# MCG-NJU/MotionRAG

Hardware: AMD Instinct MI355X
Metric: denoise_step_frames_per_sec (higher is better)
Workload: dtype bf16

## Files before the change

### include/mrag_hip.h

```cpp
#ifndef MRAG_HIP_H
#define MRAG_HIP_H

#include <stdint.h>

#ifdef __cplusplus
extern "C" {
#endif

#define MRAG_OK 0
#define MRAG_EINVAL (-1)
#define MRAG_ENOTSUP (-2)

int mrag_abi_version(void);
const char* mrag_target_arch(void);
const char* mrag_source_hash(void);

enum mrag_kernel_id {
  MRAG_K_GEMM_W4 = 0,
  MRAG_K_GEMM_W4_QKNORM_ROPE,
  MRAG_K_GEMM_W4_GEGLU,
  MRAG_K_GEMM_256x256,
  MRAG_K_GEMM_256x320,
  MRAG_K_GEMM_256x128,
  MRAG_K_GEMM_128x128,
// ... 69 lines not shown
  float qk_eps, q_premul;
  int32_t qk_first;
  int32_t tuning;
  int32_t geglu_act;
  void* workspace;
  float acc_scale;
  int64_t workspace_bytes;
  int64_t w_batch_stride;
  const void* a_ln_gamma; const void* a_ln_beta;
  float a_ln_eps; int32_t a_ln;
} mrag_gemm_args;
enum { MRAG_GEMM_TUNE_NO_WIDE = 1, MRAG_GEMM_TUNE_NO_STAGED = 2, MRAG_GEMM_TUNE_GEGLU_NO_STAGED = 4, MRAG_GEMM_TUNE_STREAMK = 8,
       MRAG_GEMM_TUNE_NO_W4 = 1 << 16,
       MRAG_GEMM_TUNE_NO_SKINNY = 1 << 17,
       MRAG_GEMM_TUNE_SKINNY_8 = 1 << 18,
       MRAG_GEMM_TUNE_TAIL_RECT = 1 << 19  };

int mrag_gemm_bf16(void* stream, const mrag_gemm_args* args);
int64_t mrag_gemm_workspace_bytes(int64_t M, int64_t N, int64_t K);

int mrag_quant_rows_e4m3(void* stream, const void* x, void* x8, int32_t* exp, int64_t M, int64_t K, int64_t ldx, int64_t ld8);

typedef struct mrag_gemm_fp8_args {
  const void* A8;
  const void* W8;
  const int32_t* a_exp;
  const int32_t* w_exp;
  const void* bias;
  void* C;
  const void* resid;
  const void* gate0;
  const void* gate1;
  int64_t M, N, K;
// ... 267 lines not shown
```

### motionrag_amd/attn_processor.py

```python
from __future__ import annotations

from typing import Optional

import torch
from torch import nn

from . import ops
from .layers import WeightCache, linear_resid


def packed_score_layout(heads: int, keys: int):
    tiles32 = -(-(heads * 32) // 256)
    for c in range(keys + (keys & 1), 32, 2):
        if -(-((heads - 1) * c + 32) // 256) < tiles32 and all(((c * h) & 7) + keys <= 32 for h in range(min(heads, 8))):
            return c, -(-((heads - 1) * c + 32) // 256) * 256
    return 32, heads * 32


PACK_SCORE_BLOCKS = True
FOLD_IP_QUERY = True


class Attention(nn.Module):

    def __init__(self, query_dim: int, cross_attention_dim: Optional[int] = None, heads: int = 8, dim_head: int = 64, bias: bool = False,
                 out_bias: bool = True, qk_norm: Optional[str] = None, eps: float = 1e-5, processor=None):
        super().__init__()
        inner = heads * dim_head
        self.heads, self.inner_dim = heads, inner
        self.is_cross_attention = cross_attention_dim is not None
        kv_dim = cross_attention_dim if cross_attention_dim is not None else query_dim
        self.to_q = nn.Linear(query_dim, inner, bias=bias)
        self.to_k = nn.Linear(kv_dim, inner, bias=bias)
        self.to_v = nn.Linear(kv_dim, inner, bias=bias)
        self.to_out = nn.ModuleList([nn.Linear(inner, query_dim, bias=out_bias), nn.Dropout(0.0)])
# ... 23 lines not shown

def _joint_sdpa(q, k, v, fp8_attn: bool):
    if fp8_attn and ops.fp8_joint_attention_supported(q.shape[1], k.shape[1]):
        return ops.joint_attention_fp8(q, k, v, q_prescaled=True)
    return ops.attention(q, k, v, q_prescaled=True)


def joint_attention_core(attn, proc, x: torch.Tensor, text_len: int, rope, ip_hidden_states: Optional[torch.Tensor], scale: float, sp=None,
                         fp8_qkv: bool = False, fp8_attn: bool = False):
    B, S, D = x.shape
    H = attn.heads
    fw = proc._fused
    qkv_lins = (attn.to_q, attn.to_k, attn.to_v)
    wqkv, bqkv = fw.get("qkv", tuple(m.weight for m in qkv_lins) + tuple(m.bias for m in qkv_lins),
                        lambda: (_cat_weights(qkv_lins), _cat_weights(qkv_lins, "bias")))
    cos = sin = None
    if rope is not None:
        cos, sin = fw.get("rope", (rope[0], rope[1]), lambda: tuple(t.to(device=x.device, dtype=torch.float32).contiguous() for t in rope[:2]))
        if getattr(attn, "is_cross_attention", False):
            raise NotImplementedError("RoPE on Q only (is_cross_attention=True) is not used by CogVideoX attn1")
    nq, nk = getattr(attn, "norm_q", None), getattr(attn, "norm_k", None)
    if sp is not None:
        o = _sharded_attention(attn, x, wqkv, bqkv, H, nq, nk, cos, sin, text_len, sp, fp8_attn)
        return _motion_branch(attn, proc, o, ip_hidden_states, scale)
    if fp8_qkv:
        w8, w_exp = fw.get("qkv8", tuple(m.weight for m in qkv_lins), lambda: ops.quant_rows_e4m3(wqkv))
        qkv = ops.linear_fp8(x, w8, w_exp, bqkv)
        ops.qknorm_rope_(qkv, H, nq.weight if nq is not None else None, nq.bias if nq is not None else None, nk.weight if nk is not None else None,
                         nk.bias if nk is not None else None, cos, sin, text_len, eps=nq.eps if nq is not None else 1e-6, q_premul=ops.LOG2E * 64 ** -0.5)
        q5 = qkv.view(B, S, 3, H, 64)
        o = _joint_sdpa(q5[:, :, 0], q5[:, :, 1], q5[:, :, 2], fp8_attn)
        return _motion_branch(attn, proc, o, ip_hidden_states, scale)
    qkv = ops.qkv_linear_qknorm_rope(x, wqkv, bqkv, H, nq.weight if nq is not None else None, nq.bias if nq is not None else None,
                                     nk.weight if nk is not None else None, nk.bias if nk is not None else None, cos, sin, text_len,
                                     eps=nq.eps if nq is not None else 1e-6, q_premul=ops.LOG2E * 64 ** -0.5)
    q5 = qkv.view(B, S, 3, H, 64)
    o = _joint_sdpa(q5[:, :, 0], q5[:, :, 1], q5[:, :, 2], fp8_attn)
    return _motion_branch(attn, proc, o, ip_hidden_states, scale)


def _sharded_attention(attn, x, wqkv, bqkv, H, nq, nk, cos, sin, text_len, sp, fp8_attn=False):
    B, S, D = x.shape
    qn = dict(eps=nq.eps if nq is not None else 1e-6, q_premul=ops.LOG2E * 64 ** -0.5)
    gq, bq, gk, bk = (nq.weight if nq is not None else None, nq.bias if nq is not None else None,
                      nk.weight if nk is not None else None, nk.bias if nk is not None else None)
    try:
        kv = ops.qkv_linear_qknorm_rope(x, wqkv[D:], bqkv[D:] if bqkv is not None else None, H, gq, bq, gk, bk, cos, sin, text_len, first=1, **qn)
    except NotImplementedError:
        qkv = ops.qkv_linear_qknorm_rope(x, wqkv, bqkv, H, gq, bq, gk, bk, cos, sin, text_len, **qn)
        g = sp.all_gather_rows_async(qkv[..., D:].contiguous()).wait().view(B, -1, 2, H, 64)
# ... 156 lines not shown
```

### motionrag_amd/csrc/gemm_bf16.hip

```cpp
#include "gemm_common.h"

namespace {

inline bool skinny_applies(const mrag_gemm_args* a, int epi) {
  const long long row_tiles = (a->M + SKM_ROWS - 1) / SKM_ROWS;
  return a->M <= 256 && row_tiles * a->N * a->K <= 8LL * 4096 * 2048 && a->K >= 256 && a->N >= 256 &&
         !(a->tuning & MRAG_GEMM_TUNE_NO_SKINNY) && ((a->tuning >> 4) & 0xf) == 0 &&
         (epi == MRAG_EPI_NONE || epi == MRAG_EPI_GELU_TANH || epi == MRAG_EPI_GELU_ERF || epi == MRAG_EPI_SILU || epi == MRAG_EPI_RESID) &&
         (!a->bias || (((uintptr_t)a->bias) & 7) == 0);
}

inline bool k320_applies(const mrag_gemm_args* a, int epi) {
  return a->K == 320 && a->N % 320 == 0 && a->N <= 960 && a->M >= 16384 && (epi == MRAG_EPI_NONE || epi == MRAG_EPI_RESID) &&
         !(a->tuning & (MRAG_GEMM_TUNE_NO_WIDE | MRAG_GEMM_TUNE_NO_STAGED | MRAG_GEMM_TUNE_GEGLU_NO_STAGED | MRAG_GEMM_TUNE_STREAMK)) &&
         rows_16B_aligned(a->C, a->ldc, a->resid, a->ldr) && (!a->bias || (((uintptr_t)a->bias) & 7) == 0);
}

}

extern "C" int mrag_gemm_bf16(void* stream, const mrag_gemm_args* a) {
  if (!a || !a->A || !a->W || !a->C) return MRAG_EINVAL;
  if (a->M <= 0 || a->N <= 0 || a->K <= 0) return MRAG_EINVAL;
  if (a->K % 64 != 0 || a->N % 4 != 0) return MRAG_ENOTSUP;
  if (a->epilogue == MRAG_EPI_GEGLU && a->N % 32 != 0) return MRAG_ENOTSUP;
  if (a->lda % 8 != 0 || a->ldw % 8 != 0 || a->ldc % 4 != 0) return MRAG_EINVAL;
  if (((uintptr_t)a->A | (uintptr_t)a->W) & 15) return MRAG_EINVAL;
  if ((uintptr_t)a->C & 7) return MRAG_EINVAL;
  if ((a->epilogue == MRAG_EPI_RESID || a->epilogue == MRAG_EPI_GATE_RESID) &&
      (!a->resid || a->ldr % 4 != 0 || ((uintptr_t)a->resid & 7)))
    return MRAG_EINVAL;
  if (a->epilogue == MRAG_EPI_GATE_RESID &&
      (!a->gate0 || !a->gate1 || a->rows_per_batch <= 0 || a->gate_stride % 4 != 0)) return MRAG_EINVAL;
  GemmP p{};
  p.A = (const bf16_t*)a->A; p.W = (const bf16_t*)a->W; p.bias = (const bf16_t*)a->bias;
  p.C = (bf16_t*)a->C; p.resid = (const bf16_t*)a->resid;
// ... 3 lines not shown
  p.acc_scale = a->acc_scale == 0.0f ? 1.0f : a->acc_scale;
  if (a->w_batch_stride < 0 || a->w_batch_stride % 8 != 0) return MRAG_EINVAL;
  if (a->a_ln != 0 && a->a_ln != 1) return MRAG_EINVAL;
  if (a->a_ln) {
    if ((((uintptr_t)a->a_ln_gamma | (uintptr_t)a->a_ln_beta) & 15) || a->K > 8192) return MRAG_EINVAL;
    p.lna = 1; p.lna_g = (const bf16_t*)a->a_ln_gamma; p.lna_b = (const bf16_t*)a->a_ln_beta; p.lna_eps = a->a_ln_eps;
  }
  p.w_bstride = a->w_batch_stride;
  if (a->epilogue == MRAG_EPI_GEGLU && a->geglu_act != 0 && a->geglu_act != 1) return MRAG_EINVAL;
  if (a->epilogue == MRAG_EPI_QKNORM_ROPE) {
    if (a->qk_dmodel <= 0 || a->qk_dmodel % 64 != 0 || a->N % a->qk_dmodel != 0 || a->qk_first < 0 || a->qk_first + a->N / a->qk_dmodel > 3 ||
        a->rows_per_batch <= 0) return MRAG_EINVAL;
    if ((a->rope_cos != nullptr) != (a->rope_sin != nullptr) || (((uintptr_t)a->rope_cos | (uintptr_t)a->rope_sin) & 15)) return MRAG_EINVAL;
    if (((uintptr_t)a->q_gamma | (uintptr_t)a->q_beta | (uintptr_t)a->k_gamma | (uintptr_t)a->k_beta) & 15) return MRAG_EINVAL;
    p.qg = (const bf16_t*)a->q_gamma; p.qb = (const bf16_t*)a->q_beta; p.kg = (const bf16_t*)a->k_gamma; p.kb = (const bf16_t*)a->k_beta;
    p.rcos = a->rope_cos; p.rsin = a->rope_sin; p.qk_D = a->qk_dmodel; p.rope_text_len = a->rope_text_len; p.qk_first = a->qk_first; p.qk_eps = a->qk_eps; p.q_premul = a->q_premul;
  }
  hipStream_t s = (hipStream_t)stream;
  const long long t256 = ((a->M + 255) / 256) * ((a->N + 255) / 256);
  p.tuning = a->tuning;
  const int epi = (a->epilogue == MRAG_EPI_GEGLU && a->geglu_act == 1) ? EPI_GEGLU_TANH : a->epilogue;
  if (const int cfg = (a->tuning >> 4) & 0xf) {
    if (cfg == 1 && t256 >= 192) return launch_tiled(s, p, epi, TILE_256x256_W16, nullptr);
    if (cfg == 2) return launch_tiled(s, p, epi, TILE_128x128, nullptr);
    if (cfg == 4 || (cfg == 3 && t256 >= 192)) {
      const int rc = launch_w4(s, p, epi);
      if (rc != MRAG_ENOTSUP) return rc;
    }
  }
  if (a->w_batch_stride != 0) {
    if (epi != MRAG_EPI_NONE || a->N % 128 != 0 || a->K < 320 || a->rows_per_batch <= 0 || a->M % a->rows_per_batch != 0 || a->ldc % 8 != 0 || (((uintptr_t)a->C) & 15) ||
        (a->tuning & (MRAG_GEMM_TUNE_NO_W4 | MRAG_GEMM_TUNE_NO_STAGED)))
      return MRAG_ENOTSUP;
    return launch_w4(s, p, epi);
  }
  if (a->a_ln) return skinny_applies(a, epi) ? launch_skinny(s, p, epi) : MRAG_ENOTSUP;
  if (skinny_applies(a, epi)) return launch_skinny(s, p, epi);
  if (k320_applies(a, epi)) return launch_k320(s, p, epi);
  const bool w4_ok = t256 >= 192 && !(a->tuning & (MRAG_GEMM_TUNE_NO_W4 | MRAG_GEMM_TUNE_NO_STAGED | MRAG_GEMM_TUNE_STREAMK | MRAG_GEMM_TUNE_NO_WIDE)) && a->N % 128 == 0 &&
// ... 16 lines not shown
    if (pl.use && a->workspace_bytes >= (int64_t)pl.bytes) {
      if ((uintptr_t)a->workspace & 15) return MRAG_EINVAL;
      p.sk_ticket = (unsigned*)a->workspace;
      p.sk_part = (float*)((char*)a->workspace + SK_TICKET_BYTES);
      p.sk_main = pl.n_main; p.sk_rem = pl.rem; p.sk_units = pl.units; p.sk_maxparts = pl.maxparts;
      const hipError_t e = hipMemsetAsync(a->workspace, 0, SK_TICKET_BYTES, s);
      if (e != hipSuccess) return (int)e;
      const int rc = launch_tiled(s, p, epi, TILE_256x256, &pl);
      if (rc != MRAG_ENOTSUP) return rc;
    }
  }
  if (t256 >= 192) return launch_tiled(s, p, epi, TILE_256x256, nullptr);
  return launch_tiled(s, p, epi, TILE_128x128, nullptr);
}

extern "C" int64_t mrag_gemm_workspace_bytes(int64_t M, int64_t N, int64_t K) {
  if (M <= 0 || N <= 0 || K <= 0 || K % 64 != 0) return 0;
  if (wide_n_pays(N)) return 0;
  const SkPlan pl = plan_streamk(M, N, K);
  return pl.use ? (int64_t)pl.bytes : 0;
}
```

### motionrag_amd/csrc/gemm_common.h

```cpp
#pragma once
#include <type_traits>
#include "common.h"
#include "../../include/mrag_hip.h"

namespace {

struct GemmP {
  const bf16_t* A; const bf16_t* W; const bf16_t* bias; bf16_t* C; const bf16_t* resid;
  const bf16_t* gate0; const bf16_t* gate1;
  long long M, N, K, lda, ldw, ldc, ldr, rows_per_batch, split, gate_stride;
  int tiles_m, tiles_n, group_m, staged, tuning;
  const bf16_t* qg; const bf16_t* qb; const bf16_t* kg; const bf16_t* kb; const float* rcos; const float* rsin;
  long long qk_D; int rope_text_len, qk_first; float qk_eps, q_premul;
  int cv_H, cv_W, cv_Hi, cv_Wi, cv_Ho, cv_Wo, cv_stride, cv_up, cv_ctiles, cv_T, cv_pad;
  long long cv_C, cv_HW;
  float acc_scale;
  float* sk_part; unsigned* sk_ticket;
  int sk_main, sk_rem, sk_units, sk_maxparts;
  const bf16_t* lna_g; const bf16_t* lna_b; float lna_eps; int lna;
  int tile_limit;
  int wb_tiles_m;
  long long w_bstride;
  int cv_lds;
  int cv_tf;
  long long cv_fs;
};

constexpr int SK_CUS = 256, SK_TICKET_BYTES = 1024;
constexpr int SK_FLAG_OFF = 8 * 128 * 144;
constexpr int SKM_ROWS = 32;

__device__ __forceinline__ float sum8_dpp(float x) {
  x += __int_as_float(__builtin_amdgcn_update_dpp(0, __float_as_int(x), 0xB1, 0xF, 0xF, true));
  x += __int_as_float(__builtin_amdgcn_update_dpp(0, __float_as_int(x), 0x4E, 0xF, 0xF, true));
  x += __int_as_float(__builtin_amdgcn_update_dpp(0, __float_as_int(x), 0x141, 0xF, 0xF, true));
  return x;
}

__device__ __forceinline__ u32x4 qk_row_math(u32x4 val, const bool has_gamma, const bool has_beta, const float (&gam)[8], const float (&bet)[8], const float eps,
                                             const bool has_rope, const bool vid, const f32x4 (&t4)[4], const bool premul_on, const float premul) {
// ... 7 lines not shown
    sum = sum8_dpp(sum);
    const float mean = sum * (1.0f / 64.0f);
    float sq = 0.f;
#pragma unroll
    for (int e = 0; e < 8; ++e) { v[e] -= mean; sq += v[e] * v[e]; }
    sq = sum8_dpp(sq);
    const float rstd = rsqrtf(sq * (1.0f / 64.0f) + eps);
#pragma unroll
    for (int e = 0; e < 8; ++e) v[e] = v[e] * rstd * gam[e];
    if (has_beta) {
#pragma unroll
      for (int e = 0; e < 8; ++e) v[e] += bet[e];
    }
  }
  if (has_rope) {
    const float cc[8] = {t4[0][0], t4[0][1], t4[0][2], t4[0][3], t4[1][0], t4[1][1], t4[1][2], t4[1][3]};
    const float ss[8] = {t4[2][0], t4[2][1], t4[2][2], t4[2][3], t4[3][0], t4[3][1], t4[3][2], t4[3][3]};
#pragma unroll
    for (int i2 = 0; i2 < 4; ++i2) {
      const float a = v[2 * i2], b2 = v[2 * i2 + 1];
      const float oa = a * cc[2 * i2] - b2 * ss[2 * i2];
      const float ob = b2 * cc[2 * i2 + 1] + a * ss[2 * i2 + 1];
      v[2 * i2] = vid ? oa : a;
      v[2 * i2 + 1] = vid ? ob : b2;
    }
  }
  if (premul_on) {
#pragma unroll
    for (int e = 0; e < 8; ++e) v[e] *= premul;
  }
#pragma unroll
  for (int e = 0; e < 4; ++e) val[e] = pack_bf2(v[2 * e], v[2 * e + 1]);
  return val;
}

constexpr int EPI_GEGLU_TANH = 8;
template <int EPI>
constexpr bool is_geglu = (EPI == MRAG_EPI_GEGLU || EPI == EPI_GEGLU_TANH);

template <int EPI>
__device__ __forceinline__ float epi_act(float v) {
  if constexpr (EPI == MRAG_EPI_GELU_TANH) return gelu_tanh_f(v);
  else if constexpr (EPI == MRAG_EPI_GELU_ERF) return gelu_erf_f(v);
  else if constexpr (EPI == MRAG_EPI_SILU) return silu_f(v);
  else return v;
}


// ... 76 lines not shown
```

### motionrag_amd/csrc/gemm_w4.hip

```cpp
#include "gemm_common.h"

namespace {

__device__ __forceinline__ int lane_id_here() {
  int l;
  asm volatile("v_mbcnt_lo_u32_b32 %0, -1, 0\n\tv_mbcnt_hi_u32_b32 %0, -1, %0" : "=v"(l));
  return l;
}
__device__ __forceinline__ int opaque_sign(int x) {
  asm volatile("" : "+v"(x));
  return x;
}

template <int EPI>
__device__ __forceinline__ void epilogue_w4(const GemmP& p, char* smem, f32x4 (&acc)[8][8], const long long bm0, const long long bn0, const int wave, const int wrow0,
                                            const int wcol0, const long long Mend) {
  constexpr bool HAS_R = (EPI == MRAG_EPI_GATE_RESID || EPI == MRAG_EPI_RESID), HAS_G = (EPI == MRAG_EPI_GATE_RESID), QK = (EPI == MRAG_EPI_QKNORM_ROPE);
  const int lane = lane_id_here();
  const int frag_row = opaque_sign(lane & 15), frag_q = lane >> 4;
  const long long n0 = bn0 + wcol0 + frag_q * 4;
  const long long m0 = bm0 + wrow0;
  long long g_b = 0, g_pos = 0;
  if constexpr (HAS_G || QK) {
    g_b = m0 / p.rows_per_batch;
    g_pos = m0 - g_b * p.rows_per_batch;
  }
  if (m0 >= Mend || bn0 + wcol0 >= p.N) return;
  const int mrows = (int)(Mend - m0 < 128 ? Mend - m0 : 128);
  bool fast = p.staged && bn0 + wcol0 + 128 <= p.N;
// ... 26 lines not shown
  };
  if (fast) {
    u32x2 bias[8], gate[8];
#pragma unroll
    for (int j = 0; j < 8; ++j) {
      bias[j] = p.bias ? *(const u32x2*)(p.bias + n0 + 16 * j) : u32x2{0u, 0u};
      if constexpr (HAS_G) gate[j] = *(const u32x2*)((g_pos < p.split ? p.gate0 : p.gate1) + g_b * p.gate_stride + n0 + 16 * j);
      else gate[j] = u32x2{0u, 0u};
    }
    const int r4 = lane >> 4, chunk = opaque_sign(lane & 15);
    const bf16_t* rbase = HAS_R ? p.resid + m0 * p.ldr + n0 : nullptr;
    bf16_t* cbase = p.C + (m0 + r4) * p.ldc + (bn0 + wcol0 + chunk * 8);
    char* wput = smem + 131072 + wave * 8192 + frag_row * 256 + (frag_q & 1) * 8;
    const char* wget = smem + 131072 + wave * 8192 + r4 * 256;
    const int xput = frag_q >> 1;
    int qk_which = 2;
    bool has_rope = false;
    const bf16_t *gm = nullptr, *bt = nullptr;
    float gam[8], bet[8];
    f32x4 qk_tab[QK ? 3 : 1][4];
    unsigned qk_video = 0;
    auto qk_fetch = [&](const int st) __attribute__((always_inline)) {
      if constexpr (QK) {
        const int row = 4 * st + r4;
        long long pos = g_pos + (row < mrows ? row : mrows - 1);
        while (pos >= p.rows_per_batch) pos -= p.rows_per_batch;
        const int rp = (int)pos - p.rope_text_len;
        if (rp >= 0) qk_video |= 1u << st;
        const long long ro = (long long)opaque_sign(rp > 0 ? rp : 0) * 64 + opaque_sign(chunk & 7) * 8;
        f32x4(&dst)[4] = qk_tab[st % 3];
        dst[0] = *(const f32x4*)(p.rcos + ro); dst[1] = *(const f32x4*)(p.rcos + ro + 4);
        dst[2] = *(const f32x4*)(p.rsin + ro); dst[3] = *(const f32x4*)(p.rsin + ro + 4);
      }
    };
    if constexpr (QK) {
      qk_which = p.qk_first + (int)((bn0 + wcol0) / p.qk_D);
      has_rope = p.rcos != nullptr && qk_which < 2;
#pragma unroll
      for (int e = 0; e < 8; ++e) { gam[e] = 1.f; bet[e] = 0.f; }
      if (qk_which < 2) {
        gm = qk_which ? p.kg : p.qg;
        bt = qk_which ? p.kb : p.qb;
        const int d0 = (chunk & 7) * 8;
        if (gm) {
          const u32x4 graw = *(const u32x4*)(gm + d0);
#pragma unroll
          for (int e = 0; e < 4; ++e) { gam[2 * e] = __uint_as_float(graw[e] << 16); gam[2 * e + 1] = __uint_as_float(graw[e] & 0xffff0000u); }
          if (bt) {
            const u32x4 braw = *(const u32x4*)(bt + d0);
#pragma unroll
            for (int e = 0; e < 4; ++e) { bet[2 * e] = __uint_as_float(braw[e] << 16); bet[2 * e + 1] = __uint_as_float(braw[e] & 0xffff0000u); }
          }
        }
      }
      if (has_rope) { qk_fetch(0); qk_fetch(1); qk_fetch(2); }
    }
    constexpr int RD = 2;
    u32x2 rr[RD][8];
    auto fetch = [&](const int i, const int slot) __attribute__((always_inline)) {
      if constexpr (HAS_R) {
        const int row = 16 * i + frag_row;
        const bf16_t* rrow = rbase + (long long)(row < mrows ? row : mrows - 1) * p.ldr;
#pragma unroll
        for (int j = 0; j < 8; ++j) rr[slot][j] = *(const u32x2*)(rrow + 16 * j);
      }
    };
    auto put = [&](const int i) __attribute__((always_inline)) {
#pragma unroll
      for (int j = 0; j < 8; ++j) {
        u32x2 out = acc_math(i, j, bias[j], gate[j]);
// ... 5 lines not shown
      u32x4 val[4];
#pragma unroll
      for (int q = 0; q < 4; ++q) val[q] = *(const u32x4*)(wget + (i & 1) * 4096 + q * 1024 + ((chunk ^ (q * 4 + r4)) * 16));
#pragma unroll
      for (int q = 0; q < 4; ++q) {
        if constexpr (QK) {
          const int st = 4 * i + q;
          if (qk_which < 2) {
            val[q] = qk_row_math(val[q], gm != nullptr, bt != nullptr, gam, bet, p.qk_eps, has_rope, (qk_video >> st) & 1u, qk_tab[st % 3], qk_which == 0 && p.q_premul != 1.0f, p.q_premul);
            if (has_rope && st + 3 < 32) qk_fetch(st + 3);
          }
        }
        if (16 * i + 4 * q + r4 < mrows) *(u32x4*)(cbase + (long long)(16 * i + 4 * q) * p.ldc) = val[q];
      }
    };
#pragma unroll
    for (int i = 0; i < RD - 1; ++i) fetch(i, i);
#pragma unroll
    for (int i = 0; i < 8; ++i) {
      __builtin_amdgcn_sched_barrier(0);
      if (i + RD - 1 < 8) fetch(i + RD - 1, (i + RD - 1) % RD);
      put(i);
      if (i > 0) get_store(i - 1);
    }
    __builtin_amdgcn_sched_barrier(0);
    get_store(7);
    return;
  }
  if constexpr (QK) return;
  auto ncol = [&](const int j) __attribute__((always_inline)) { const long long n = n0 + 16 * j; return n < p.N ? n : p.N - 4; };
// ... 78 lines not shown
__device__ __forceinline__ void static_for(F&& f) {
  if constexpr (N > 0) {
    static_for<N - 1>(f);
    f(std::integral_constant<int, N - 1>{});
  }
}

__device__ __forceinline__ void tile_coords(const GemmP& p, const int L, int& tile_m, int& tile_n) {
  const int gw = p.group_m * p.tiles_n;
  const int first_m = (L / gw) * p.group_m;
  const int gsz = min(p.tiles_m - first_m, p.group_m);
  tile_m = first_m + (L % gw) % gsz;
  tile_n = (L % gw) / gsz;
}

template <int EPI, bool WB = false>
__global__ __launch_bounds__(256) void gemm_w4_kernel(const GemmP p) {
  extern __shared__ __attribute__((aligned(16))) char smem[];
  constexpr unsigned STAGE = 65536, WOFF = 32768;
  const int lane = threadIdx.x & 63;
  const int wave_s = __builtin_amdgcn_readfirstlane(threadIdx.x >> 6), wm = wave_s >> 1, wn = wave_s & 1;
  const int tiles = p.tile_limit, nk = (int)(p.K / 64), G = (int)gridDim.x;
  auto tile_origin = [&](const int tm, long long& bm0, long long& m_end, long long& w_off) __attribute__((always_inline)) {
    if constexpr (WB) {
      const int b = tm / p.wb_tiles_m;
      bm0 = (long long)b * p.rows_per_batch + (long long)(tm - b * p.wb_tiles_m) * 256;
      m_end = (long long)(b + 1) * p.rows_per_batch;
      w_off = (long long)b * p.w_bstride;
    } else {
      bm0 = (long long)tm * 256; m_end = p.M; w_off = 0;
    }
// ... 99 lines not shown
#pragma unroll
    for (int i = 0; i < 8; ++i)
#pragma unroll
      for (int j = 0; j < 8; ++j) acc[i][j] = f32x4{0.f, 0.f, 0.f, 0.f};
    asm volatile("s_nop 4" ::: "memory");
    for (int t = 0; t < nk; ++t, ++g) {
      kstep(g, !(t == 0 && r > 0));
      advance();
    }
    asm volatile("s_waitcnt vmcnt(0) lgkmcnt(0)\n\ts_nop 15\n\ts_nop 15\n\ts_nop 7" ::: "memory");
    int tm, tn;
    tile_coords(p, L, tm, tn);
    long long e_bm0, e_mend, e_woff;
    tile_origin(tm, e_bm0, e_mend, e_woff);
    if constexpr (is_geglu<EPI>) epilogue_w4_geglu<EPI>(p, smem, acc, e_bm0, (long long)tn * 256, wave_s, wm * 128, wn * 128);
    else epilogue_w4<EPI>(p, smem, acc, e_bm0, (long long)tn * 256, wave_s, wm * 128, wn * 128, e_mend);
  }
#undef MRAG_W4_MF
#undef MRAG_W4_RD
#undef MRAG_W4_LGKM0
}

struct TailRect { bool use = false; int limit = 0; long long r0 = 0, c0 = 0; };
inline TailRect plan_tail_rect(const GemmP& p, int epi) {
  TailRect t;
  const long long tiles = (long long)p.tiles_m * p.tiles_n;
  if (p.wb_tiles_m || !tail_rect_wanted(tiles, epi, p.tuning)) return t;
  const int rem = (int)(tiles % SK_CUS);
  const int first_m = ((p.tiles_m - 1) / p.group_m) * p.group_m, gsz = p.tiles_m - first_m;
  const int ncols = (rem + gsz - 1) / gsz;
  if (ncols > p.tiles_n) return t;
  t.use = true;
  t.limit = (int)(tiles - (long long)gsz * ncols);
  t.r0 = (long long)first_m * 256; t.c0 = (long long)(p.tiles_n - ncols) * 256;
  return t;
}

}

extern "C" int launch_w4(hipStream_t s, const GemmP& p0, int epi) {
  if (256LL * (p0.lda > p0.ldw ? p0.lda : p0.ldw) * 2 >= (1LL << 32)) return MRAG_ENOTSUP;
  GemmP p = p0;
  const bool wb = p.w_bstride != 0;
  if (wb) {
    if (epi != MRAG_EPI_NONE || p.rows_per_batch <= 0 || p.M % p.rows_per_batch != 0) return MRAG_ENOTSUP;
    p.wb_tiles_m = (int)((p.rows_per_batch + 255) / 256);
    p.tiles_m = (int)(p.M / p.rows_per_batch) * p.wb_tiles_m;
  } else {
    p.wb_tiles_m = 0;
    p.tiles_m = (int)((p.M + 255) / 256);
  }
  p.tiles_n = (int)((p.N + 255) / 256);
// ... 8 lines not shown
  int rc;
  switch (epi) {
    case MRAG_EPI_NONE:
      rc = wb ? launch_dyn_lds(gemm_w4_kernel<MRAG_EPI_NONE, true>, grid, block, lds, s, p) : launch_dyn_lds(gemm_w4_kernel<MRAG_EPI_NONE>, grid, block, lds, s, p);
      break;
    case MRAG_EPI_GELU_TANH: rc = launch_dyn_lds(gemm_w4_kernel<MRAG_EPI_GELU_TANH>, grid, block, lds, s, p); break;
    case MRAG_EPI_RESID: rc = launch_dyn_lds(gemm_w4_kernel<MRAG_EPI_RESID>, grid, block, lds, s, p); break;
    case MRAG_EPI_GATE_RESID: rc = launch_dyn_lds(gemm_w4_kernel<MRAG_EPI_GATE_RESID>, grid, block, lds, s, p); break;
    case MRAG_EPI_GEGLU:
    case EPI_GEGLU_TANH:
      if (!p.staged || p.N % 128 != 0) return MRAG_ENOTSUP;
      rc = epi == MRAG_EPI_GEGLU ? launch_dyn_lds(gemm_w4_kernel<MRAG_EPI_GEGLU>, grid, block, lds, s, p) : launch_dyn_lds(gemm_w4_kernel<EPI_GEGLU_TANH>, grid, block, lds, s, p);
      break;
    case MRAG_EPI_QKNORM_ROPE:
      if (!p.staged || p.N % 128 != 0 || p.qk_D % 128 != 0) return MRAG_ENOTSUP;
      rc = launch_dyn_lds(gemm_w4_kernel<MRAG_EPI_QKNORM_ROPE>, grid, block, lds, s, p);
      break;
    default: return MRAG_ENOTSUP;
  }
  if (rc != MRAG_OK) return rc;
  MRAG_COUNT(epi == MRAG_EPI_QKNORM_ROPE ? MRAG_K_GEMM_W4_QKNORM_ROPE : (epi == MRAG_EPI_GEGLU || epi == EPI_GEGLU_TANH) ? MRAG_K_GEMM_W4_GEGLU : wb ? MRAG_K_GEMM_W4_BATCHED_W : MRAG_K_GEMM_W4);
  if (tail.use) {
    GemmP t = p0;
    t.A = p0.A + tail.r0 * p0.lda; t.W = p0.W + tail.c0 * p0.ldw; t.C = p0.C + tail.r0 * p0.ldc + tail.c0;
    if (p0.bias) t.bias = p0.bias + tail.c0;
    if (p0.resid) t.resid = p0.resid + tail.r0 * p0.ldr + tail.c0;
    t.M = p0.M - tail.r0; t.N = p0.N - tail.c0;
    rc = launch_tiled(s, t, epi, TILE_128x128, nullptr);
    if (rc != MRAG_OK) return rc;
    MRAG_COUNT(MRAG_K_GEMM_W4_TAIL_RECT);
  }
  return MRAG_OK;
}
```

### motionrag_amd/csrc/pointwise.hip

```cpp
#include "common.h"
#include "../../include/mrag_hip.h"

namespace {

constexpr int kMaxBlocks = 2048;

__device__ __forceinline__ void unpack8(const u32x4 r, float* f) {
#pragma unroll
  for (int i = 0; i < 4; ++i) {
    f[2 * i] = __uint_as_float(r[i] << 16);
    f[2 * i + 1] = __uint_as_float(r[i] & 0xffff0000u);
  }
}
__device__ __forceinline__ u32x4 pack8(const float* f) {
  u32x4 r;
#pragma unroll
  for (int i = 0; i < 4; ++i) r[i] = pack_bf2(f[2 * i], f[2 * i + 1]);
  return r;
}

inline unsigned grid_for(long long work_items) {
  long long b = (work_items + 255) / 256;
  if (b > kMaxBlocks) b = kMaxBlocks;
  if (b < 1) b = 1;
// ... 368 lines not shown
  MRAG_LAUNCH(weighted_sum_kernel, grid, dim3(256), 0, (hipStream_t)stream, (const bf16_t*)x, w, (bf16_t*)out, K, n / 8, div);
  MRAG_LAUNCH_CHECK();
  return MRAG_OK;
}

extern "C" int mrag_softmax_rows_bf16(void* stream, const void* x, void* y, int64_t rows, int64_t cols, int64_t ldx, int64_t ldy, float scale) {
  if (!x || !y || rows <= 0 || cols <= 0 || ldx < cols || ldy < cols || !(scale > 0.f)) return MRAG_EINVAL;
  if ((((uintptr_t)x | (uintptr_t)y) & 15) || (ldx % 8) || (ldy % 8)) return MRAG_EINVAL;
  if (rows > 0x7fffffffLL) return MRAG_EINVAL;
  MRAG_LAUNCH(softmax_rows_kernel, dim3((unsigned)rows), dim3(256), 0, (hipStream_t)stream, (const bf16_t*)x, (bf16_t*)y, (long long)cols, (long long)ldx, (long long)ldy, scale);
  MRAG_LAUNCH_CHECK();
  return MRAG_OK;
}

namespace {
__global__ __launch_bounds__(256) void blend_tile_kernel(bf16_t* tile, const bf16_t* up, const bf16_t* left, int T, int th, int tw, int C, int uh, int lw,
                                                         int ev, int eh) {
  const long long total = (long long)T * th * tw * C;
  for (long long i = (long long)blockIdx.x * 256 + threadIdx.x; i < total; i += (long long)gridDim.x * 256) {
    const int c = (int)(i % C);
    long long r = i / C;
    const int x = (int)(r % tw); r /= tw;
    const int y = (int)(r % th);
    const int t = (int)(r / th);
    const bool bv = up && y < ev, bh = left && x < eh;
    if (!bv && !bh) continue;
    float v = bf2f(tile[i]);
    if (bv) {
      const float w = (float)y / (float)ev;
      v = bf2f(f2bf(bf2f(up[(((long long)t * uh + (uh - ev + y)) * tw + x) * C + c]) * (1.f - w) + v * w));
// ... 35 lines not shown
```

### motionrag_amd/ops.py

```python
from __future__ import annotations

import ctypes
from typing import Optional

import torch

from . import _lib
from ._lib import AttnArgs, AttnVarlenArgs, ConvArgs, ConvFp8Args, FfFusedArgs, GemmArgs, GemmFp8Args, GroupNormArgs, LnArgs, QkNormRopeArgs, check


def _header(prefix: str, *names: str):
    return (_lib.CONSTANTS["MRAG_" + prefix + n] for n in names)


EPI_NONE, EPI_GELU_TANH, EPI_GELU_ERF, EPI_RESID, EPI_GATE_RESID, EPI_SILU, EPI_GEGLU, EPI_QKNORM_ROPE = _header(
    "EPI_", "NONE", "GELU_TANH", "GELU_ERF", "RESID", "GATE_RESID", "SILU", "GEGLU", "QKNORM_ROPE")
GEMM_TUNE_NO_WIDE, GEMM_TUNE_NO_STAGED, GEMM_TUNE_GEGLU_NO_STAGED, GEMM_TUNE_STREAMK, GEMM_TUNE_NO_W4, GEMM_TUNE_NO_SKINNY, GEMM_TUNE_TAIL_RECT = _header(
    "GEMM_TUNE_", "NO_WIDE", "NO_STAGED", "GEGLU_NO_STAGED", "STREAMK", "NO_W4", "NO_SKINNY", "TAIL_RECT")
ATTN_TUNE_NO_TINY, ATTN_TUNE_LEGACY, ATTN_TUNE_FP8_QUANT_ONLY = _header("ATTN_TUNE_", "NO_TINY", "LEGACY", "FP8_QUANT_ONLY")
CONV_3X3, CONV_T3 = _header("CONV_", "3X3", "T3")
FF_FUSED_ROWS = _lib.CONSTANTS["MRAG_FF_FUSED_ROWS"]
LOG2E = 1.4426950408889634

TUNING = {"gemm": 0, "attn": 0, "attn_no_split": False, "no_qkv_fuse": False, "no_batched_w": False, "gn_fold": False}


class HipOnly(RuntimeError):
    """Raised when an op is handed a tensor that is not on the GPU (no CPU fallback exists)."""


def _launch_counts(entry: str, n: int) -> list:
    buf = (ctypes.c_uint64 * n)()
    getattr(_lib.lib(), entry)(buf, n)
    return [int(v) for v in buf]


def dispatch_counts() -> dict:
    L = _lib.lib()
    n = L.mrag_dispatch_counts(None, 0)
    buf = (ctypes.c_uint64 * n)()
    L.mrag_dispatch_counts(buf, n)
    return {L.mrag_dispatch_name(i).decode(): int(buf[i]) for i in range(n)}


class dispatched:

    def __enter__(self):
        self._before = dispatch_counts()
        self.counts = {}
        return self

    def __exit__(self, *exc):
        after = dispatch_counts()
        self.counts = {k: after[k] - self._before[k] for k in after if after[k] != self._before[k]}
        return False


# ... 354 lines not shown
        raise ValueError("qkv must be a contiguous [B, S, 3*H*64]")
    a = QkNormRopeArgs()
    a.qkv, a.q_gamma, a.q_beta, a.k_gamma, a.k_beta = _p(qkv), _p(q_gamma), _p(q_beta), _p(k_gamma), _p(k_beta)
    if cos is not None:
        _dev(cos, torch.float32, "cos"); _dev(sin, torch.float32, "sin")
        if tuple(cos.shape) != (S - text_len, 64) or not cos.is_contiguous() or not sin.is_contiguous():
            raise ValueError("cos/sin must be contiguous [S - text_len, 64] fp32")
        a.cos, a.sin = _p(cos), _p(sin)
    a.B, a.S, a.H, a.text_len, a.eps, a.q_premul = B, S, H, text_len, eps, q_premul
    check(_lib.lib().mrag_qknorm_rope_bf16(_stream(), ctypes.byref(a)), "mrag_qknorm_rope_bf16")
    return qkv


def qkv_linear_qknorm_rope(x: torch.Tensor, weight: torch.Tensor, bias: Optional[torch.Tensor], H: int, q_gamma, q_beta, k_gamma, k_beta,
                           cos: Optional[torch.Tensor], sin: Optional[torch.Tensor], text_len: int, eps: float = 1e-6, q_premul: float = 1.0,
                           first: int = 0, out: Optional[torch.Tensor] = None) -> torch.Tensor:
    _dev(x, name="x"); _dev(weight, name="weight")
    B, S, K = x.shape
    N = weight.shape[0]
    D = H * 64
    if N % D or first + N // D > 3 or weight.shape[1] != K or not x.is_contiguous() or K % 64 != 0:
        raise ValueError("qkv_linear_qknorm_rope: x [B, S, K] contiguous, weight [n*H*64, K] with first + n <= 3, K % 64 == 0")
    if out is None:
        out = torch.empty(B, S, N, dtype=torch.bfloat16, device=x.device)
    a = GemmArgs()
    a.A, a.W, a.bias, a.C = _p(x), _p(weight), _p(bias), _p(out)
    a.M, a.N, a.K, a.lda, a.ldw, a.ldc = B * S, N, K, K, weight.stride(0), N
    a.epilogue, a.rows_per_batch, a.rope_text_len, a.qk_dmodel, a.qk_eps, a.q_premul, a.qk_first = EPI_QKNORM_ROPE, S, text_len, D, eps, q_premul, first
    a.q_gamma, a.q_beta, a.k_gamma, a.k_beta = _p(q_gamma), _p(q_beta), _p(k_gamma), _p(k_beta)
    if cos is not None:
        _dev(cos, torch.float32, "cos"); _dev(sin, torch.float32, "sin")
        if tuple(cos.shape) != (S - text_len, 64) or not cos.is_contiguous() or not sin.is_contiguous():
            raise ValueError("cos/sin must be contiguous [S - text_len, 64] fp32")
        a.rope_cos, a.rope_sin = _p(cos), _p(sin)
    a.tuning = TUNING["gemm"]
    _gemm_workspace(a, x.device)
    rc = _lib.MRAG_ENOTSUP if TUNING["no_qkv_fuse"] else _lib.lib().mrag_gemm_bf16(_stream(), ctypes.byref(a))
    if rc == _lib.MRAG_ENOTSUP:
        if first != 0 or N != 3 * D:
            raise NotImplementedError("the two-kernel fallback needs the whole fused [Q | K | V] buffer")
        linear(x, weight, bias, out=out)
        return qknorm_rope_(out, H, q_gamma, q_beta, k_gamma, k_beta, cos, sin, text_len, eps=eps, q_premul=q_premul)
    check(rc, "mrag_gemm_bf16")
    return out


def fp8_launch_counts() -> dict:
    return dict(zip(("gemm", "quant"), _launch_counts("mrag_fp8_launch_counts", 2)))


def fp8_linear_supported(N: int, K: int) -> bool:
    return N > 0 and K > 0 and K % 128 == 0 and N % 16 == 0


def quant_rows_e4m3(x: torch.Tensor, out: Optional[tuple] = None):
    _dev(x, name="x")
    x2 = _rows(x)
    M, K = x2.shape
    if K % 16 != 0 or x2.stride(0) % 8 != 0 or x2.data_ptr() % 16 != 0:
# ... 701 lines not shown
```

Measured before the change: 91.73.

## Use deduplicated interleaved RoPE pair table in fused QKV GEMM epilogue

```diff
diff --git a/include/mrag_hip.h b/include/mrag_hip.h
--- a/include/mrag_hip.h
+++ b/include/mrag_hip.h
@@ -107,9 +107,13 @@
        MRAG_GEMM_TUNE_NO_W4 = 1 << 16,
        MRAG_GEMM_TUNE_NO_SKINNY = 1 << 17,
        MRAG_GEMM_TUNE_SKINNY_8 = 1 << 18,
-       MRAG_GEMM_TUNE_TAIL_RECT = 1 << 19  };
+       MRAG_GEMM_TUNE_TAIL_RECT = 1 << 19 ,
+       MRAG_GEMM_TUNE_NO_ROPE_PAIRS = 1 << 20  };
 
 int mrag_gemm_bf16(void* stream, const mrag_gemm_args* args);
+int mrag_gemm_bf16_rope_pairs(void* stream, const mrag_gemm_args* args, const float* rope_pairs);
+int mrag_gemm_rope_pairs_launch_counts(uint64_t* out_host, int32_t n);
+int mrag_rope_pairs_f32(void* stream, const float* cos, const float* sin, float* pairs, int32_t* mismatch, int64_t rows);
 int64_t mrag_gemm_workspace_bytes(int64_t M, int64_t N, int64_t K);
 
 int mrag_quant_rows_e4m3(void* stream, const void* x, void* x8, int32_t* exp, int64_t M, int64_t K, int64_t ldx, int64_t ld8);
diff --git a/motionrag_amd/attn_processor.py b/motionrag_amd/attn_processor.py
--- a/motionrag_amd/attn_processor.py
+++ b/motionrag_amd/attn_processor.py
@@ -19,6 +19,7 @@
 
 PACK_SCORE_BLOCKS = True
 FOLD_IP_QUERY = True
+_ROPE_PAIRS = WeightCache()
 
 
 class Attention(nn.Module):
@@ -72,9 +73,12 @@
     qkv_lins = (attn.to_q, attn.to_k, attn.to_v)
     wqkv, bqkv = fw.get("qkv", tuple(m.weight for m in qkv_lins) + tuple(m.bias for m in qkv_lins),
                         lambda: (_cat_weights(qkv_lins), _cat_weights(qkv_lins, "bias")))
-    cos = sin = None
+    cos = sin = pairs = None
     if rope is not None:
-        cos, sin = fw.get("rope", (rope[0], rope[1]), lambda: tuple(t.to(device=x.device, dtype=torch.float32).contiguous() for t in rope[:2]))
+        def build_rope():
+            cs = tuple(t.to(device=x.device, dtype=torch.float32).contiguous() for t in rope[:2])
+            return cs + (_ROPE_PAIRS.get("pairs", cs, lambda: ops.rope_pairs(*cs)),)
+        cos, sin, pairs = fw.get("rope", (rope[0], rope[1]), build_rope)
         if getattr(attn, "is_cross_attention", False):
             raise NotImplementedError("RoPE on Q only (is_cross_attention=True) is not used by CogVideoX attn1")
     nq, nk = getattr(attn, "norm_q", None), getattr(attn, "norm_k", None)
@@ -91,7 +95,7 @@
         return _motion_branch(attn, proc, o, ip_hidden_states, scale)
     qkv = ops.qkv_linear_qknorm_rope(x, wqkv, bqkv, H, nq.weight if nq is not None else None, nq.bias if nq is not None else None,
                                      nk.weight if nk is not None else None, nk.bias if nk is not None else None, cos, sin, text_len,
-                                     eps=nq.eps if nq is not None else 1e-6, q_premul=ops.LOG2E * 64 ** -0.5)
+                                     eps=nq.eps if nq is not None else 1e-6, q_premul=ops.LOG2E * 64 ** -0.5, rope_pairs=pairs)
     q5 = qkv.view(B, S, 3, H, 64)
     o = _joint_sdpa(q5[:, :, 0], q5[:, :, 1], q5[:, :, 2], fp8_attn)
     return _motion_branch(attn, proc, o, ip_hidden_states, scale)
diff --git a/motionrag_amd/csrc/gemm_bf16.hip b/motionrag_amd/csrc/gemm_bf16.hip
--- a/motionrag_amd/csrc/gemm_bf16.hip
+++ b/motionrag_amd/csrc/gemm_bf16.hip
@@ -16,9 +16,7 @@
          rows_16B_aligned(a->C, a->ldc, a->resid, a->ldr) && (!a->bias || (((uintptr_t)a->bias) & 7) == 0);
 }
 
-}
-
-extern "C" int mrag_gemm_bf16(void* stream, const mrag_gemm_args* a) {
+int gemm_dispatch(void* stream, const mrag_gemm_args* a, const float* rope_pairs) {
   if (!a || !a->A || !a->W || !a->C) return MRAG_EINVAL;
   if (a->M <= 0 || a->N <= 0 || a->K <= 0) return MRAG_EINVAL;
   if (a->K % 64 != 0 || a->N % 4 != 0) return MRAG_ENOTSUP;
@@ -52,6 +50,8 @@
     if ((a->rope_cos != nullptr) != (a->rope_sin != nullptr) || (((uintptr_t)a->rope_cos | (uintptr_t)a->rope_sin) & 15)) return MRAG_EINVAL;
     if (((uintptr_t)a->q_gamma | (uintptr_t)a->q_beta | (uintptr_t)a->k_gamma | (uintptr_t)a->k_beta) & 15) return MRAG_EINVAL;
     p.qg = (const bf16_t*)a->q_gamma; p.qb = (const bf16_t*)a->q_beta; p.kg = (const bf16_t*)a->k_gamma; p.kb = (const bf16_t*)a->k_beta;
+    if (rope_pairs && (!a->rope_cos || ((uintptr_t)rope_pairs & 15))) return MRAG_EINVAL;
+    p.rpairs = (a->tuning & MRAG_GEMM_TUNE_NO_ROPE_PAIRS) ? nullptr : rope_pairs;
     p.rcos = a->rope_cos; p.rsin = a->rope_sin; p.qk_D = a->qk_dmodel; p.rope_text_len = a->rope_text_len; p.qk_first = a->qk_first; p.qk_eps = a->qk_eps; p.q_premul = a->q_premul;
   }
   hipStream_t s = (hipStream_t)stream;
@@ -61,6 +61,7 @@
   if (const int cfg = (a->tuning >> 4) & 0xf) {
     if (cfg == 1 && t256 >= 192) return launch_tiled(s, p, epi, TILE_256x256_W16, nullptr);
     if (cfg == 2) return launch_tiled(s, p, epi, TILE_128x128, nullptr);
+    if (cfg == 5) return launch_tiled(s, p, epi, TILE_256x256, nullptr);
     if (cfg == 4 || (cfg == 3 && t256 >= 192)) {
       const int rc = launch_w4(s, p, epi);
       if (rc != MRAG_ENOTSUP) return rc;
@@ -107,6 +108,15 @@
   return launch_tiled(s, p, epi, TILE_128x128, nullptr);
 }
 
+}
+
+extern "C" int mrag_gemm_bf16(void* stream, const mrag_gemm_args* a) { return gemm_dispatch(stream, a, nullptr); }
+
+extern "C" int mrag_gemm_bf16_rope_pairs(void* stream, const mrag_gemm_args* a, const float* rope_pairs) {
+  if (rope_pairs && (!a || a->epilogue != MRAG_EPI_QKNORM_ROPE)) return MRAG_EINVAL;
+  return gemm_dispatch(stream, a, rope_pairs);
+}
+
 extern "C" int64_t mrag_gemm_workspace_bytes(int64_t M, int64_t N, int64_t K) {
   if (M <= 0 || N <= 0 || K <= 0 || K % 64 != 0) return 0;
   if (wide_n_pays(N)) return 0;
diff --git a/motionrag_amd/csrc/gemm_common.h b/motionrag_amd/csrc/gemm_common.h
--- a/motionrag_amd/csrc/gemm_common.h
+++ b/motionrag_amd/csrc/gemm_common.h
@@ -24,6 +24,7 @@
   int cv_lds;
   int cv_tf;
   long long cv_fs;
+  const float* rpairs;
 };
 
 constexpr int SK_CUS = 256, SK_TICKET_BYTES = 1024;
@@ -61,6 +62,7 @@
     }
   }
   if (has_rope) {
+#pragma clang fp contract(off)
     const float cc[8] = {t4[0][0], t4[0][1], t4[0][2], t4[0][3], t4[1][0], t4[1][1], t4[1][2], t4[1][3]};
     const float ss[8] = {t4[2][0], t4[2][1], t4[2][2], t4[2][3], t4[3][0], t4[3][1], t4[3][2], t4[3][3]};
 #pragma unroll
@@ -79,6 +81,11 @@
 #pragma unroll
   for (int e = 0; e < 4; ++e) val[e] = pack_bf2(v[2 * e], v[2 * e + 1]);
   return val;
+}
+__device__ __forceinline__ u32x4 qk_row_math_pairs(u32x4 val, const bool has_gamma, const bool has_beta, const float (&gam)[8], const float (&bet)[8], const float eps,
+                                                   const bool has_rope, const bool vid, const f32x4 c4, const f32x4 s4, const bool premul_on, const float premul) {
+  const f32x4 t4[4] = {f32x4{c4[0], c4[0], c4[1], c4[1]}, f32x4{c4[2], c4[2], c4[3], c4[3]}, f32x4{s4[0], s4[0], s4[1], s4[1]}, f32x4{s4[2], s4[2], s4[3], s4[3]}};
+  return qk_row_math(val, has_gamma, has_beta, gam, bet, eps, has_rope, vid, t4, premul_on, premul);
 }
 
 constexpr int EPI_GEGLU_TANH = 8;
diff --git a/motionrag_amd/csrc/gemm_w4.hip b/motionrag_amd/csrc/gemm_w4.hip
--- a/motionrag_amd/csrc/gemm_w4.hip
+++ b/motionrag_amd/csrc/gemm_w4.hip
@@ -12,7 +12,7 @@
   return x;
 }
 
-template <int EPI>
+template <int EPI, bool PAIRS = false>
 __device__ __forceinline__ void epilogue_w4(const GemmP& p, char* smem, f32x4 (&acc)[8][8], const long long bm0, const long long bn0, const int wave, const int wrow0,
                                             const int wcol0, const long long Mend) {
   constexpr bool HAS_R = (EPI == MRAG_EPI_GATE_RESID || EPI == MRAG_EPI_RESID), HAS_G = (EPI == MRAG_EPI_GATE_RESID), QK = (EPI == MRAG_EPI_QKNORM_ROPE);
@@ -69,11 +69,16 @@
     char* wput = smem + 131072 + wave * 8192 + frag_row * 256 + (frag_q & 1) * 8;
     const char* wget = smem + 131072 + wave * 8192 + r4 * 256;
     const int xput = frag_q >> 1;
+    const unsigned c_row = (unsigned)p.ldc * 2u, c_voff = (unsigned)r4 * c_row + (unsigned)chunk * 16u;
+    const auto c_rsrc = __builtin_amdgcn_make_buffer_rsrc((void*)(PAIRS ? p.C + m0 * p.ldc + (bn0 + wcol0) : nullptr), 0, PAIRS ? (int)((unsigned)mrows * c_row) : 0, 0x00020000);
     int qk_which = 2;
     bool has_rope = false;
     const bf16_t *gm = nullptr, *bt = nullptr;
     float gam[8], bet[8];
-    f32x4 qk_tab[QK ? 3 : 1][4];
+    f32x4 qk_tab[QK && !PAIRS ? 3 : 1][4];
+    f32x4 qk_half[PAIRS ? 3 : 1][4];
+    int pr_off = 0;
+    if constexpr (PAIRS) pr_off = opaque_sign((chunk & 7) * 8 + (chunk >> 3) * 4);
     unsigned qk_video = 0;
     auto qk_fetch = [&](const int st) __attribute__((always_inline)) {
       if constexpr (QK) {
@@ -88,9 +93,22 @@
         dst[2] = *(const f32x4*)(p.rsin + ro); dst[3] = *(const f32x4*)(p.rsin + ro + 4);
       }
     };
+    auto qk_fetch_group = [&](const int gi) __attribute__((always_inline)) {
+      if constexpr (PAIRS) {
+#pragma unroll
+        for (int q = 0; q < 4; ++q) {
+          const int st = 4 * gi + q, row = 4 * st + r4;
+          int pos = (int)g_pos + (row < mrows ? row : mrows - 1);
+          pos -= pos >= (int)p.rows_per_batch ? (int)p.rows_per_batch : 0;
+          const int rp = pos - p.rope_text_len;
+          qk_video |= rp >= 0 ? 1u << st : 0u;
+          qk_half[gi % 3][q] = *(const f32x4*)(p.rpairs + ((long long)opaque_sign(rp > 0 ? rp : 0) * 64 + pr_off));
+        }
+      }
+    };
     if constexpr (QK) {
       qk_which = p.qk_first + (int)((bn0 + wcol0) / p.qk_D);
-      has_rope = p.rcos != nullptr && qk_which < 2;
+      has_rope = (PAIRS || p.rcos != nullptr) && qk_which < 2;
 #pragma unroll
       for (int e = 0; e < 8; ++e) { gam[e] = 1.f; bet[e] = 0.f; }
       if (qk_which < 2) {
@@ -108,7 +126,9 @@
           }
         }
       }
-      if (has_rope) { qk_fetch(0); qk_fetch(1); qk_fetch(2); }
+      if constexpr (!PAIRS) {
+        if (has_rope) { qk_fetch(0); qk_fetch(1); qk_fetch(2); }
+      }
     }
     constexpr int RD = 2;
     u32x2 rr[RD][8];
@@ -144,6 +164,45 @@
         if (16 * i + 4 * q + r4 < mrows) *(u32x4*)(cbase + (long long)(16 * i + 4 * q) * p.ldc) = val[q];
       }
     };
+    if constexpr (PAIRS) {
+      auto get_store_pairs = [&](const int i, auto ROPE) __attribute__((always_inline)) {
+        u32x4 val[4];
+#pragma unroll
+        for (int q = 0; q < 4; ++q) val[q] = *(const u32x4*)(wget + (i & 1) * 4096 + q * 1024 + ((chunk ^ (q * 4 + r4)) * 16));
+#pragma unroll
+        for (int q = 0; q < 4; ++q) {
+          if constexpr (decltype(ROPE)::value) {
+            const f32x4 own = qk_half[i % 3][q];
+            f32x4 c4, s4;
+#pragma unroll
+            for (int e = 0; e < 4; ++e) {
+              const int x = __float_as_int(own[e]);
+              c4[e] = __int_as_float(__builtin_amdgcn_update_dpp(x, x, 0x128, 0xF, 0xC, false));
+              s4[e] = __int_as_float(__builtin_amdgcn_update_dpp(x, x, 0x128, 0xF, 0x3, false));
+            }
+            val[q] = qk_row_math_pairs(val[q], gm != nullptr, bt != nullptr, gam, bet, p.qk_eps, true, (qk_video >> (4 * i + q)) & 1u, c4, s4, qk_which == 0 && p.q_premul != 1.0f, p.q_premul);
+          }
+          __builtin_amdgcn_raw_buffer_store_b128(val[q], c_rsrc, (int)(c_voff + (unsigned)(16 * i + 4 * q) * c_row), 0, 0);
+        }
+      };
+      auto rows_loop = [&](auto ROPE) __attribute__((always_inline)) {
+        if constexpr (decltype(ROPE)::value) { qk_fetch_group(0); qk_fetch_group(1); }
+#pragma unroll
+        for (int i = 0; i < 8; ++i) {
+          __builtin_amdgcn_sched_barrier(0);
+          if constexpr (decltype(ROPE)::value) {
+            if (i >= 1 && i + 1 < 8) qk_fetch_group(i + 1);
+          }
+          put(i);
+          if (i > 0) get_store_pairs(i - 1, ROPE);
+        }
+        __builtin_amdgcn_sched_barrier(0);
+        get_store_pairs(7, ROPE);
+      };
+      if (qk_which < 2) rows_loop(std::true_type{});
+      else rows_loop(std::false_type{});
+      return;
+    }
 #pragma unroll
     for (int i = 0; i < RD - 1; ++i) fetch(i, i);
 #pragma unroll
@@ -252,7 +311,7 @@
   tile_n = (L % gw) / gsz;
 }
 
-template <int EPI, bool WB = false>
+template <int EPI, bool WB = false, bool PAIRS = false>
 __global__ __launch_bounds__(256) void gemm_w4_kernel(const GemmP p) {
   extern __shared__ __attribute__((aligned(16))) char smem[];
   constexpr unsigned STAGE = 65536, WOFF = 32768;
@@ -382,7 +441,7 @@
     long long e_bm0, e_mend, e_woff;
     tile_origin(tm, e_bm0, e_mend, e_woff);
     if constexpr (is_geglu<EPI>) epilogue_w4_geglu<EPI>(p, smem, acc, e_bm0, (long long)tn * 256, wave_s, wm * 128, wn * 128);
-    else epilogue_w4<EPI>(p, smem, acc, e_bm0, (long long)tn * 256, wave_s, wm * 128, wn * 128, e_mend);
+    else epilogue_w4<EPI, PAIRS>(p, smem, acc, e_bm0, (long long)tn * 256, wave_s, wm * 128, wn * 128, e_mend);
   }
 #undef MRAG_W4_MF
 #undef MRAG_W4_RD
@@ -404,6 +463,13 @@
   return t;
 }
 
+unsigned long long rope_pairs_launches;
+
+}
+
+extern "C" int mrag_gemm_rope_pairs_launch_counts(uint64_t* out_host, int32_t n) {
+  if (out_host && n > 0) out_host[0] = __atomic_load_n(&rope_pairs_launches, __ATOMIC_RELAXED);
+  return 1;
 }
 
 extern "C" int launch_w4(hipStream_t s, const GemmP& p0, int epi) {
@@ -442,11 +508,14 @@
       break;
     case MRAG_EPI_QKNORM_ROPE:
       if (!p.staged || p.N % 128 != 0 || p.qk_D % 128 != 0) return MRAG_ENOTSUP;
-      rc = launch_dyn_lds(gemm_w4_kernel<MRAG_EPI_QKNORM_ROPE>, grid, block, lds, s, p);
+      if (p.rows_per_batch < 128 || 128LL * p.ldc * 2 >= (1LL << 31)) p.rpairs = nullptr;
+      rc = p.rpairs ? launch_dyn_lds(gemm_w4_kernel<MRAG_EPI_QKNORM_ROPE, false, true>, grid, block, lds, s, p)
+                    : launch_dyn_lds(gemm_w4_kernel<MRAG_EPI_QKNORM_ROPE>, grid, block, lds, s, p);
       break;
     default: return MRAG_ENOTSUP;
   }
   if (rc != MRAG_OK) return rc;
+  if (epi == MRAG_EPI_QKNORM_ROPE && p.rpairs) (void)__atomic_fetch_add(&rope_pairs_launches, 1ull, __ATOMIC_RELAXED);
   MRAG_COUNT(epi == MRAG_EPI_QKNORM_ROPE ? MRAG_K_GEMM_W4_QKNORM_ROPE : (epi == MRAG_EPI_GEGLU || epi == EPI_GEGLU_TANH) ? MRAG_K_GEMM_W4_GEGLU : wb ? MRAG_K_GEMM_W4_BATCHED_W : MRAG_K_GEMM_W4);
   if (tail.use) {
     GemmP t = p0;
diff --git a/motionrag_amd/csrc/pointwise.hip b/motionrag_amd/csrc/pointwise.hip
--- a/motionrag_amd/csrc/pointwise.hip
+++ b/motionrag_amd/csrc/pointwise.hip
@@ -406,6 +406,28 @@
 }
 
 namespace {
+__global__ void rope_pairs_kernel(const float* cs, const float* sn, float* pairs, int* mismatch, long long chunks) {
+  for (long long i = (long long)blockIdx.x * blockDim.x + threadIdx.x; i < chunks; i += (long long)gridDim.x * blockDim.x) {
+    const u32x4 c0 = *(const u32x4*)(cs + i * 8), c1 = *(const u32x4*)(cs + i * 8 + 4);
+    const u32x4 s0 = *(const u32x4*)(sn + i * 8), s1 = *(const u32x4*)(sn + i * 8 + 4);
+    *(u32x4*)(pairs + i * 8) = u32x4{c0[0], c0[2], c1[0], c1[2]};
+    *(u32x4*)(pairs + i * 8 + 4) = u32x4{s0[0], s0[2], s1[0], s1[2]};
+    if (c0[0] != c0[1] || c0[2] != c0[3] || c1[0] != c1[1] || c1[2] != c1[3] || s0[0] != s0[1] || s0[2] != s0[3] || s1[0] != s1[1] || s1[2] != s1[3]) *mismatch = 1;
+  }
+}
+}
+
+extern "C" int mrag_rope_pairs_f32(void* stream, const float* cos, const float* sin, float* pairs, int32_t* mismatch, int64_t rows) {
+  if (!cos || !sin || !pairs || !mismatch || rows <= 0 || rows > (1LL << 40)) return MRAG_EINVAL;
+  if ((((uintptr_t)cos | (uintptr_t)sin | (uintptr_t)pairs) & 15) || ((uintptr_t)mismatch & 3)) return MRAG_EINVAL;
+  const hipError_t e = hipMemsetAsync(mismatch, 0, sizeof(int32_t), (hipStream_t)stream);
+  if (e != hipSuccess) return (int)e;
+  MRAG_LAUNCH(rope_pairs_kernel, dim3(grid_for(rows * 8)), dim3(256), 0, (hipStream_t)stream, cos, sin, pairs, (int*)mismatch, (long long)(rows * 8));
+  MRAG_LAUNCH_CHECK();
+  return MRAG_OK;
+}
+
+namespace {
 __global__ __launch_bounds__(256) void blend_tile_kernel(bf16_t* tile, const bf16_t* up, const bf16_t* left, int T, int th, int tw, int C, int uh, int lw,
                                                          int ev, int eh) {
   const long long total = (long long)T * th * tw * C;
diff --git a/motionrag_amd/ops.py b/motionrag_amd/ops.py
--- a/motionrag_amd/ops.py
+++ b/motionrag_amd/ops.py
@@ -17,6 +17,7 @@
     "EPI_", "NONE", "GELU_TANH", "GELU_ERF", "RESID", "GATE_RESID", "SILU", "GEGLU", "QKNORM_ROPE")
 GEMM_TUNE_NO_WIDE, GEMM_TUNE_NO_STAGED, GEMM_TUNE_GEGLU_NO_STAGED, GEMM_TUNE_STREAMK, GEMM_TUNE_NO_W4, GEMM_TUNE_NO_SKINNY, GEMM_TUNE_TAIL_RECT = _header(
     "GEMM_TUNE_", "NO_WIDE", "NO_STAGED", "GEGLU_NO_STAGED", "STREAMK", "NO_W4", "NO_SKINNY", "TAIL_RECT")
+GEMM_TUNE_NO_ROPE_PAIRS, = _header("GEMM_TUNE_", "NO_ROPE_PAIRS")
 ATTN_TUNE_NO_TINY, ATTN_TUNE_LEGACY, ATTN_TUNE_FP8_QUANT_ONLY = _header("ATTN_TUNE_", "NO_TINY", "LEGACY", "FP8_QUANT_ONLY")
 CONV_3X3, CONV_T3 = _header("CONV_", "3X3", "T3")
 FF_FUSED_ROWS = _lib.CONSTANTS["MRAG_FF_FUSED_ROWS"]
@@ -40,7 +41,9 @@
     n = L.mrag_dispatch_counts(None, 0)
     buf = (ctypes.c_uint64 * n)()
     L.mrag_dispatch_counts(buf, n)
-    return {L.mrag_dispatch_name(i).decode(): int(buf[i]) for i in range(n)}
+    counts = {L.mrag_dispatch_name(i).decode(): int(buf[i]) for i in range(n)}
+    counts["GEMM_W4_QKNORM_ROPE_PAIRS"] = _launch_counts("mrag_gemm_rope_pairs_launch_counts", 1)[0]
+    return counts
 
 
 class dispatched:
@@ -425,7 +428,7 @@
 
 def qkv_linear_qknorm_rope(x: torch.Tensor, weight: torch.Tensor, bias: Optional[torch.Tensor], H: int, q_gamma, q_beta, k_gamma, k_beta,
                            cos: Optional[torch.Tensor], sin: Optional[torch.Tensor], text_len: int, eps: float = 1e-6, q_premul: float = 1.0,
-                           first: int = 0, out: Optional[torch.Tensor] = None) -> torch.Tensor:
+                           first: int = 0, out: Optional[torch.Tensor] = None, rope_pairs: Optional[torch.Tensor] = None) -> torch.Tensor:
     _dev(x, name="x"); _dev(weight, name="weight")
     B, S, K = x.shape
     N = weight.shape[0]
@@ -444,9 +447,13 @@
         if tuple(cos.shape) != (S - text_len, 64) or not cos.is_contiguous() or not sin.is_contiguous():
             raise ValueError("cos/sin must be contiguous [S - text_len, 64] fp32")
         a.rope_cos, a.rope_sin = _p(cos), _p(sin)
+    if rope_pairs is not None:
+        _dev(rope_pairs, torch.float32, "rope_pairs")
+        if cos is None or tuple(rope_pairs.shape) != (S - text_len, 8, 8) or not rope_pairs.is_contiguous():
+            raise ValueError("rope_pairs must be the contiguous [S - text_len, 8, 8] fp32 table that rope_pairs(cos, sin) returns")
     a.tuning = TUNING["gemm"]
     _gemm_workspace(a, x.device)
-    rc = _lib.MRAG_ENOTSUP if TUNING["no_qkv_fuse"] else _lib.lib().mrag_gemm_bf16(_stream(), ctypes.byref(a))
+    rc = _lib.MRAG_ENOTSUP if TUNING["no_qkv_fuse"] else _lib.lib().mrag_gemm_bf16_rope_pairs(_stream(), ctypes.byref(a), _p(rope_pairs))
     if rc == _lib.MRAG_ENOTSUP:
         if first != 0 or N != 3 * D:
             raise NotImplementedError("the two-kernel fallback needs the whole fused [Q | K | V] buffer")
@@ -454,6 +461,16 @@
         return qknorm_rope_(out, H, q_gamma, q_beta, k_gamma, k_beta, cos, sin, text_len, eps=eps, q_premul=q_premul)
     check(rc, "mrag_gemm_bf16")
     return out
+
+
+def rope_pairs(cos: torch.Tensor, sin: torch.Tensor) -> Optional[torch.Tensor]:
+    _dev(cos, torch.float32, "cos"); _dev(sin, torch.float32, "sin")
+    if cos.dim() != 2 or cos.shape[1] != 64 or sin.shape != cos.shape or cos.shape[0] < 1 or not cos.is_contiguous() or not sin.is_contiguous():
+        raise ValueError("cos/sin must be contiguous [R, 64] fp32 with R >= 1")
+    pairs = torch.empty(cos.shape[0], 8, 8, dtype=torch.float32, device=cos.device)
+    flag = torch.empty(1, dtype=torch.int32, device=cos.device)
+    check(_lib.lib().mrag_rope_pairs_f32(_stream(), _p(cos), _p(sin), _p(pairs), _p(flag), cos.shape[0]), "mrag_rope_pairs_f32")
+    return None if int(flag.item()) else pairs
 
 
 def fp8_launch_counts() -> dict:
```

Measured after the change: 92.00, median of 6. Within noise of the previous version (+0.3%).
